# mrjoshuak/go-blosc

Hardware: AMD Instinct MI355X
Metric: GB/s compress+decompress, 1 GiB float32 Shuffle+LZ4 (higher is better)
Workload: dtype u8; 1 GPU; 1024 MiB f32 frame per GPU, shuffle=1 typesize=4 + LZ4, compress then decompress, device-resident; index_trailer=True, chunk_bytes=4096, decode_entry=hb_decompress_frame_dev_hdr (header known to the host)

## Files before the change

go-blosc_amd/csrc/hb_lz4_dec.hip:

```cpp
#include "hb_lz4.h"
#include "hb_dec_common.h"

size_t hb_lz4_dec_workspace(size_t n_out) { return 256 + hb_lz4_region_workspace(n_out); }

__device__ __forceinline__ uint32_t ld32(const uint8_t *p) { return ld4u(p); }

__device__ __forceinline__ void dec_plan_check(const uint8_t *__restrict__ index, uint64_t index_bytes, uint64_t n_src, uint64_t cap,
                                               DecPlan *plan, hb_result *result) {
    plan->mode = DEC_SERIAL; plan->fail = 0; plan->nunits = 0; plan->nbytes = 0; plan->post = 0; plan->stride = 1;
    result->status = HB_OK; result->flags = 0; result->bytes = 0; result->total_bytes = 0; result->reserved = 0;
    if (!index || index_bytes < HB_IDX_HDR_BYTES + 2 * HB_IDX_ENTRY) return;
    uint32_t h[8];
    for (int i = 0; i < 8; i++) h[i] = ld32(index + 4 * i);
    if (h[0] != HB_IDX_MAGIC || h[1] != (HB_IDX_VERSION | (HB_IDX_ENTRY << 16))) return;
    if (h[7] != (h[0] ^ h[1] ^ h[2] ^ h[3] ^ h[4] ^ h[5])) return;
    const uint64_t nunits = h[2];
    if (nunits == 0 || HB_IDX_HDR_BYTES + (nunits + 1) * HB_IDX_ENTRY > index_bytes) return;
    if (h[4] != n_src || h[5] > cap) return;
    if (h[3] != HB_CHUNK || nunits != ((uint64_t)h[5] + HB_CHUNK - 1) / HB_CHUNK) return;
    plan->nunits = (uint32_t)nunits;
    plan->nbytes = h[5];
    const uint32_t m = ((uint32_t)nunits + 7u) / 8u;
    uint32_t P = m / 4u + 1u;
    for (;;) {
        uint32_t x = P, y = m;
        while (y) { const uint32_t t = x % y; x = y; y = t; }
        if (x == 1u) break;
        P++;
    }
    plan->stride = P;
    plan->mode = DEC_INDEXED;
}
__global__ void k_dec_plan(const uint8_t *__restrict__ index, uint64_t index_bytes, uint64_t n_src, uint64_t cap,
                           DecPlan *plan, hb_result *result) {
    dec_plan_check(index, index_bytes, n_src, cap, plan, result);
}

#ifndef DEC_IN_WIN
#define DEC_IN_WIN  1536u
#endif
#define DEC_IN_MARGIN 320u
#define DEC_OUT_MAX HB_CHUNK
#ifndef DEC_LEAN
#define DEC_LEAN 1
#endif
#ifndef DEC_WAVES
#define DEC_WAVES 6
#endif

struct DecCtx {
    const uint8_t *src; uint64_t n_src;
    uint8_t *dst;
    const uint8_t *ent;
    DecPlan *plan;
    uint32_t nbytes, nunits;
    int bun4, ush;
};
#if defined(LAB_DEC_FLUSH) && LAB_DEC_FLUSH == 1
#define LAB_FLUSH_USH() do { } while (0)
#elif defined(LAB_DEC_FLUSH) && LAB_DEC_FLUSH == 2
#define LAB_FLUSH_USH() do { for (uint32_t i = lane * 16u; i < outlen; i += 1024u) st16u(dst + d0 + i, *(const u32x4 *)(s_out + i)); } while (0)
#else
#define LAB_FLUSH_USH() do { \
        uint32_t i_ = lane; \
        for (; i_ + 448u < outlen; i_ += 512u) { \
            _Pragma("unroll") for (uint32_t k_ = 0; k_ < 8u; k_++) udst[(size_t)(i_ + 64u * k_) * (uint32_t)ush] = s_out[i_ + 64u * k_]; \
        } \
        for (; i_ < outlen; i_ += 64) udst[(size_t)i_ * (uint32_t)ush] = s_out[i_]; \
    } while (0)
#endif
__device__ __forceinline__ void dec_unit(const DecCtx &c, const uint32_t u, uint8_t *s_in, uint8_t *s_out, uint2 *s_tq, const int lane) {
    const uint8_t *const src = c.src; const uint64_t n_src = c.n_src; uint8_t *const dst = c.dst; const uint8_t *const ent = c.ent;
    DecPlan *const plan = c.plan; const uint32_t nbytes = c.nbytes, nunits = c.nunits; const int bun4 = c.bun4, ush = c.ush;
    const u32x4 e0 = ld16u(ent + 16 * (size_t)u), e1 = ld16u(ent + 16 * (size_t)(u + 1));
#define RFL(x) ((uint32_t)__builtin_amdgcn_readfirstlane((int)(x)))
    const uint32_t s0 = RFL(e0.x), d0 = RFL(e0.y), s1 = RFL(e1.x), d1 = RFL(e1.y), rem1 = RFL(e1.z), tok1 = RFL(e1.w);
    uint32_t rem = RFL(e0.z), tokpos = RFL(e0.w);
    const bool last = (u + 1 == nunits);
    bool ok = s0 <= s1 && s1 <= n_src && d0 <= d1 && d1 <= nbytes && (d1 - d0) <= DEC_OUT_MAX;
    if (u == 0) ok = ok && s0 == 0 && d0 == 0 && rem == HB_IDX_AT_TOKEN;
    if (last) ok = ok && s1 == n_src && d1 == nbytes;
    if (rem != HB_IDX_AT_TOKEN && tokpos >= n_src) ok = false;
    if (bun4 && ((d0 | d1) & 31u)) ok = false;
    const uint32_t ne = ush ? nbytes / (uint32_t)ush : 1u;
    const uint32_t pj = ush ? d0 / ne : 0u;
    if (ush && (pj >= (uint32_t)ush || d1 > (pj + 1u) * ne)) ok = false;
    uint8_t *const udst = ush ? dst + (size_t)(d0 - pj * ne) * (uint32_t)ush + pj : dst + d0;
    if (!ok) { if (lane == 0) atomicExch(&plan->fail, 1u); return; }
    const uint32_t slen = s1 - s0, outlen = d1 - d0;
    const uint8_t *g = src + s0;

    if (rem != HB_IDX_AT_TOKEN && rem >= outlen) {
        const uint32_t left = rem - outlen;
        bool fine = slen == outlen;
        if (last) fine = fine && left == 0 && (RFL((uint32_t)src[tokpos]) & 15u) == 0u; else fine = fine && rem1 == left && tok1 == tokpos;
        if (!fine) { if (lane == 0) atomicExch(&plan->fail, 1u); return; }
        if (ush) {
            for (uint32_t i = lane * 16u; i < outlen; i += 1024u) {
                if (i + 16u <= outlen) *(u32x4 *)(s_out + i) = ld16u(g + i);
                else for (uint32_t r = i; r < outlen; r++) s_out[r] = g[r];
            }
            wave_sync();
            LAB_FLUSH_USH();
            wave_sync();
        }
        else if (!bun4) wave_copy_g2g(dst + d0, g, outlen, lane);
        else {
            for (uint32_t w = lane; w < outlen / 32u; w += 64) {
                u32x4 oa, ob;
                bitshuffle4_window<true>(ld16u(g + 32u * w), ld16u(g + 32u * w + 16u), oa, ob);
                st16u(dst + d0 + 32u * w, oa);
                st16u(dst + d0 + 32u * w + 16u, ob);
            }
        }
        return;
    }

    const uint32_t sh = (uint32_t)((uintptr_t)g & 15u);
    uint32_t wlo = 0, staged = 0;
    int shw = 0;
    auto stage = [&](const uint32_t at) __attribute__((always_inline)) {
        wave_sync();
        const uint32_t a16 = (sh + at) & ~15u;
        const uint32_t avail = sh + slen - a16;
        const uint32_t cnt = avail < DEC_IN_WIN ? avail : DEC_IN_WIN;
        const u32x4 *ga = (const u32x4 *)(g - sh + a16);
        const uint32_t nv = (cnt + 15u) >> 4;
        for (uint32_t i = lane; i < nv; i += 64) ((u32x4 *)s_in)[i] = ga[i];
        wlo = a16 > sh ? a16 - sh : 0u;
        staged = a16 + cnt - sh;
        shw = (int)sh - (int)a16;
        wave_sync();
    };
    stage(0u);
    uint32_t tok = 0;
    if (rem != HB_IDX_AT_TOKEN) tok = RFL((uint32_t)src[tokpos]);
#define INB(i) s_in[(uint32_t)((int)(i) + shw)]
    uint32_t si = 0, di = 0;
    bool at_token = false;
    bool done = false;

    int slow = 1;
    uint32_t nq = 0;
    uint32_t last_ntok = DEC_BPERM_MIN; (void)last_ntok;
    if (rem == HB_IDX_AT_TOKEN) { rem = 0; slow = 0; }
    while (ok && !done) {
        if (slow) {
            if (slow == 2) {
                if (si >= slen) { ok = false; break; }
                tokpos = s0 + si;
                tok = RFL((uint32_t)((si >= wlo && si < staged) ? INB(si) : g[si]));
                si++;
                rem = tok >> 4;
                if (rem == 15u && !dec_read_ext(s_in, shw, wlo, staged, g, slen, si, rem, lane)) { ok = false; break; }
            }
            slow = 0;
            {
                const uint32_t take = min(rem, outlen - di);
                if (take > slen - si) { ok = false; break; }
                if (si >= wlo && si + take <= staged) { for (uint32_t i = lane; i < take; i += 64) s_out[di + i] = INB(si + i); }
                else { for (uint32_t i = lane; i < take; i += 64) s_out[di + i] = g[si + i]; }
                si += take; di += take; rem -= take;
            }
            if (rem > 0 || di == outlen) { at_token = false; done = true; break; }
            if (slen - si < 2) { ok = false; break; }
            const uint32_t b0 = RFL((uint32_t)((si >= wlo && si < staged) ? INB(si) : g[si]));
            const uint32_t b1 = RFL((uint32_t)((si + 1 >= wlo && si + 1 < staged) ? INB(si + 1) : g[si + 1]));
            const uint32_t offset = b0 | (b1 << 8);
            si += 2;
            uint32_t mlen = (tok & 15u) + 4u;
            if ((tok & 15u) == 15u && !dec_read_ext(s_in, shw, wlo, staged, g, slen, si, mlen, lane)) { ok = false; break; }
            if (offset == 0 || offset > di || mlen > outlen - di) { ok = false; break; }
            dec_match_copy(s_out, di, offset, mlen, lane);
            di += mlen;
            if (si >= wlo && si + 4u <= staged && di < outlen) {
                const uint32_t t2 = RFL((uint32_t)INB(si)), l2 = t2 >> 4;
                if (l2 < 15u && (t2 & 15u) == 15u) {
                    const uint32_t op = si + 1u + l2;
                    if (op + 3u <= staged && RFL((uint32_t)INB(op + 2u)) == 255u) slow = 2;
                }
            }
            continue;
        }
        if (nq == 0u && staged < slen && si + DEC_IN_MARGIN > staged) {
            stage(si);
        }
#if DEC_LEAN
        const bool stop = dec_fill_lean(s_in, (uint32_t)shw, staged, slen, si, nq, s_tq, lane, last_ntok);
        bool rewound = false;
        ok = dec_drain<true>(s_in, shw, s_out, outlen, 0u, di, si, nq, s_tq, stop, rewound, lane);
#else
        const bool stop = dec_fill(s_in, (uint32_t)shw, staged, slen, si, nq, s_tq, lane);
        bool rewound = false;
        ok = dec_drain(s_in, shw, s_out, outlen, 0u, di, si, nq, s_tq, stop, rewound, lane);
#endif
        if (!ok) break;
        if (rewound) { slow = 2; continue; }
        if (stop) {
            if (si == slen || di == outlen) { at_token = true; done = true; }
            else if (staged < slen && si + DEC_IN_MARGIN > staged) continue;
            else slow = 2;
        }
    }
    if (ok) {
        ok = (si == slen) && (di == outlen);
        if (last) ok = ok && (at_token || (rem == 0 && (tok & 15u) == 0u));
        else if (at_token) ok = ok && rem1 == HB_IDX_AT_TOKEN;
        else ok = ok && rem1 == rem && tok1 == tokpos;
    }
    if (!ok) { if (lane == 0) atomicExch(&plan->fail, 1u); wave_sync(); return; }
    wave_sync();
    if (bun4) {
        for (uint32_t w = lane; w < outlen / 32u; w += 64) {
            u32x4 oa, ob;
            bitshuffle4_window<true>(((const u32x4 *)s_out)[2 * w], ((const u32x4 *)s_out)[2 * w + 1], oa, ob);
            ((u32x4 *)s_out)[2 * w] = oa;
            ((u32x4 *)s_out)[2 * w + 1] = ob;
        }
        wave_sync();
    }
    if (ush) {
        LAB_FLUSH_USH();
    } else {
        uint8_t *o = dst + d0;
        uint32_t head = (uint32_t)((16u - ((uintptr_t)o & 15u)) & 15u);
        if (head > outlen) head = outlen;
        if ((uint32_t)lane < head) o[lane] = s_out[lane];
        const uint32_t body = (outlen - head) >> 4;
        if (head == 0) { for (uint32_t i = lane; i < body; i += 64) *(u32x4 *)(o + i * 16u) = *(const u32x4 *)(s_out + i * 16u); }
        else {
            for (uint32_t i = lane; i < body; i += 64) {
                const uint8_t *q = s_out + head + i * 16u;
                u32x4 v;
                v.x = (uint32_t)q[0] | ((uint32_t)q[1] << 8) | ((uint32_t)q[2] << 16) | ((uint32_t)q[3] << 24);
                v.y = (uint32_t)q[4] | ((uint32_t)q[5] << 8) | ((uint32_t)q[6] << 16) | ((uint32_t)q[7] << 24);
                v.z = (uint32_t)q[8] | ((uint32_t)q[9] << 8) | ((uint32_t)q[10] << 16) | ((uint32_t)q[11] << 24);
                v.w = (uint32_t)q[12] | ((uint32_t)q[13] << 8) | ((uint32_t)q[14] << 16) | ((uint32_t)q[15] << 24);
                *(u32x4 *)(o + head + i * 16u) = v;
            }
        }
        const uint32_t done_b = head + body * 16u;
        if (done_b + lane < outlen) o[done_b + lane] = s_out[done_b + lane];
    }
    wave_sync();
}

__global__ __launch_bounds__(64) __attribute__((amdgpu_waves_per_eu(DEC_WAVES))) void k_dec_indexed(const uint8_t *__restrict__ src, uint64_t n_src,
                                                    uint8_t *__restrict__ dst, const uint8_t *__restrict__ index,
                                                    DecPlan *plan, int bun4, int ush, uint32_t plane_mask) {
    __shared__ __attribute__((aligned(16))) uint8_t s_in[DEC_IN_WIN + 128];
    __shared__ __attribute__((aligned(16))) uint8_t s_out[DEC_OUT_MAX + 64];
    __shared__ __attribute__((aligned(16))) uint2 s_tq[DEC_LEAN ? DTQ / 4 : DTQ];
    if (plan->mode != DEC_INDEXED) return;
    const int lane = threadIdx.x;
    const uint32_t nunits = plan->nunits;
    const uint8_t *ent = index + HB_IDX_HDR_BYTES;
    const uint32_t nbytes = plan->nbytes;

    const uint32_t P = plan->stride;
    const uint32_t mgrp = (nunits + 7u) / 8u;
    for (uint32_t it = blockIdx.x; it < mgrp * 8u; it += gridDim.x) {
        uint32_t u = (uint32_t)(((uint64_t)(it >> 3) * P) % mgrp) * 8u + ((it + (it >> 3)) & 7u);
        const bool fused_order = ush && nunits % (uint32_t)ush == 0u && (gridDim.x % (8u * (uint32_t)ush) == 0u || gridDim.x >= nunits);
        if (fused_order ? it >= nunits : u >= nunits) continue;
        if (fused_order) {
            const uint32_t T = (uint32_t)ush, nblk = nunits / T;
            const uint32_t grp = it / (8u * T), r = it % (8u * T);
            uint32_t b = grp * 8u + (r & 7u), j = ((r >> 3) + it / gridDim.x) % T;
            if (grp * 8u + 8u > nblk) {
                const uint32_t k = it - grp * 8u * T, nb = nblk - grp * 8u;
                b = grp * 8u + k % nb; j = k / nb;
            }
            u = j * nblk + b;
            if (!((plane_mask >> j) & 1u)) continue;
        }
        DecCtx c; c.src = src; c.n_src = n_src; c.dst = dst; c.ent = ent; c.plan = plan; c.nbytes = nbytes; c.nunits = nunits; c.bun4 = bun4; c.ush = ush;
        dec_unit(c, u, s_in, s_out, s_tq, lane);
    }
}

__global__ __launch_bounds__(64) void k_bt_dec_plan(const DecBatchFrame *__restrict__ bf, uint32_t nframes, uint32_t *__restrict__ unit_frame, uint32_t total_units) {
    const uint32_t f = blockIdx.x;
    const DecBatchFrame b = bf[f];
    const uint32_t next = f + 1 < nframes ? bf[f + 1].unit0 : total_units;
    __shared__ uint32_t s_mode;
    if (threadIdx.x == 0) {
        dec_plan_check(b.preset == 1 ? b.index : nullptr, b.index_bytes, b.n_src, (uint64_t)b.nbytes, b.plan, b.result);
        b.plan->pad[0] = 0; b.plan->pad[1] = 0;
        if (b.plan->mode == DEC_INDEXED && (b.plan->nunits != b.nunits || b.plan->nbytes != b.nbytes)) b.plan->mode = DEC_SERIAL;
        s_mode = b.plan->mode;
    }
    __syncthreads();
    const bool indexed = s_mode == DEC_INDEXED;
    for (uint32_t u = threadIdx.x; u < next - b.unit0; u += 64) unit_frame[b.unit0 + u] = (u < b.nunits && indexed) ? f : 0xFFFFFFFFu;
}

__global__ __launch_bounds__(64) __attribute__((amdgpu_waves_per_eu(DEC_WAVES))) void k_dec_indexed_batch(const DecBatchFrame *__restrict__ bf,
                                                    const uint32_t *__restrict__ unit_frame, uint32_t total_units) {
    __shared__ __attribute__((aligned(16))) uint8_t s_in[DEC_IN_WIN + 128];
    __shared__ __attribute__((aligned(16))) uint8_t s_out[DEC_OUT_MAX + 64];
    __shared__ __attribute__((aligned(16))) uint2 s_tq[DEC_LEAN ? DTQ / 4 : DTQ];
    const int lane = threadIdx.x;
    for (uint32_t it = blockIdx.x; it < total_units; it += gridDim.x) {
        const uint32_t fid = unit_frame[it];
        if (fid == 0xFFFFFFFFu) continue;
        const DecBatchFrame &f = bf[fid];
        DecCtx c; c.src = f.src; c.n_src = f.n_src; c.dst = f.dst; c.ent = f.index + HB_IDX_HDR_BYTES; c.plan = f.plan;
        c.nbytes = f.nbytes; c.nunits = f.nunits; c.bun4 = f.bun4; c.ush = f.ush;
        uint32_t u = it - f.unit0;
        if (c.ush) {
            const uint32_t T = (uint32_t)c.ush, nblk = c.nunits / T;
            const uint32_t grp = u / (8u * T), r = u % (8u * T);
            uint32_t b = grp * 8u + (r & 7u), j = ((r >> 3) + it / gridDim.x) % T;
            if (grp * 8u + 8u > nblk) { const uint32_t k = u - grp * 8u * T, nb = nblk - grp * 8u; b = grp * 8u + k % nb; j = k / nb; }
            u = j * nblk + b;
        }
        if (u >= c.nunits) continue;
        dec_unit(c, u, s_in, s_out, s_tq, lane);
    }
}

size_t hb_lz4_dec_batch_units(int nframes, const DecBatchFrame *h, uint32_t *unit0_out) {
    uint64_t units = 0;
    for (int k = 0; k < nframes; k++) {
        const uint32_t g = h[k].ush ? 8u * (uint32_t)h[k].ush : 8u;
        units = (units + g - 1) / g * g;
        unit0_out[k] = (uint32_t)units;
        units += h[k].nunits;
    }
    return (size_t)((units + 7) / 8 * 8);
}

int hb_launch_lz4_decode_batch_indexed(int nframes, const DecBatchFrame *d_bf, uint32_t *d_unit_frame, uint32_t total_units, int any_ush, hipStream_t s) {
    hb_prof_begin("k_dec_plan", s);
    hipLaunchKernelGGL(k_bt_dec_plan, dim3((unsigned)nframes), dim3(64), 0, s, d_bf, (uint32_t)nframes, d_unit_frame, total_units);
    hb_prof_end(s);
    if (total_units) {
        unsigned grid = total_units < 256u * 256u ? total_units : 256u * 256u;
        if (any_ush && total_units > 256u * 16u) {
            const unsigned gran = 32u;
            unsigned g2 = total_units / (unsigned)any_ush / gran * gran;
            if (total_units > 256u * 64u && g2 < 256u * 64u) g2 = 256u * 64u;
            if (g2 > 256u * 256u) g2 = 256u * 256u;
            if (g2) grid = g2;
        }
        hb_prof_begin("k_dec_indexed", s);
        hipLaunchKernelGGL(k_dec_indexed_batch, dim3(grid), dim3(64), 0, s, d_bf, (const uint32_t *)d_unit_frame, total_units);
        hb_prof_end(s);
    }
    HB_HIP_TRY(hipGetLastError());
    return HB_OK;
}


__global__ __launch_bounds__(64) void k_dec_serial(const uint8_t *__restrict__ src, uint64_t n_src,
                                                   uint8_t *__restrict__ dst, uint64_t cap, DecPlan *plan,
                                                   hb_result *result, int frame, uint32_t expect, int mark_post) {
    __shared__ __attribute__((aligned(16))) uint8_t s_win[SER_WIN + 128];
    __shared__ __attribute__((aligned(16))) uint8_t s_img[SER_HIST + SER_PAGE + 1024];
    __shared__ __attribute__((aligned(16))) uint2 s_tq[DTQ];
    const int lane = threadIdx.x;
    if (plan->mode == DEC_INDEXED && !plan->fail) {
        if (lane == 0) {
            const uint64_t got = plan->nbytes;
            result->flags = 1; result->bytes = got; result->total_bytes = got;
            result->status = (frame && got != expect) ? HB_ERR_SIZE_MISMATCH : HB_OK;
        }
        return;
    }
    if (mark_post && lane == 0) plan->post = 1;
    int err;
    const uint64_t got = dec_serial_core(src, n_src, dst, cap, s_win, s_img, s_tq, lane, err);
    if (lane == 0) {
        result->flags = 0; result->total_bytes = 0;
        if (err) { result->status = HB_ERR_DECOMPRESSION_FAILED; result->bytes = 0; }
        else if (frame && got != expect) { result->status = HB_ERR_SIZE_MISMATCH; result->bytes = got; }
        else { result->status = HB_OK; result->bytes = got; }
    }
}

__global__ void k_set_result(hb_result *result, int status, uint64_t bytes) {
    result->status = status; result->flags = 0; result->bytes = bytes; result->total_bytes = bytes; result->reserved = 0;
}

int hb_launch_lz4_decode(const hb_dec_args &a, hipStream_t s) {
    if (a.memcpy_payload) {
        if (a.n != a.expect) {
            hipLaunchKernelGGL(k_set_result, dim3(1), dim3(1), 0, s, a.result, HB_ERR_SIZE_MISMATCH, (uint64_t)a.n);
        } else {
            if (a.n) HB_HIP_TRY(hipMemcpyAsync(a.dst, a.src, a.n, hipMemcpyDeviceToDevice, s));
            hipLaunchKernelGGL(k_set_result, dim3(1), dim3(1), 0, s, a.result, HB_OK, (uint64_t)a.n);
        }
        HB_HIP_TRY(hipGetLastError());
        return HB_OK;
    }
    DecPlan *plan = (DecPlan *)a.work;
    const uint8_t *index = a.index;
    size_t index_bytes = a.index_bytes;
    if (hb_lz4_region_wanted(a)) {
        const int rc = hb_launch_lz4_region_index(a, &index, &index_bytes, s);
        if (rc) return rc;
    }
    hb_prof_begin("k_dec_plan", s);
    hipLaunchKernelGGL(k_dec_plan, dim3(1), dim3(1), 0, s, index, (uint64_t)index_bytes, (uint64_t)a.n,
                       (uint64_t)a.cap, plan, a.result);
    hb_prof_end(s);
    if (index) {
        const uint64_t units = (a.cap + HB_CHUNK - 1) / HB_CHUNK;
        const uint64_t units8 = (units + 7) / 8 * 8;
        unsigned grid = (unsigned)(units8 < 8 ? 8 : (units8 < 256u * 256u ? units8 : 256u * 256u));
        if (a.fused_unshuffle_ts && units > 256u * 16u) {
            const unsigned gran = 8u * (unsigned)a.fused_unshuffle_ts;
            unsigned g2 = (unsigned)(units / (uint64_t)a.fused_unshuffle_ts) / gran * gran;
            if (units > 256u * 64u && g2 < 256u * 64u) g2 = 256u * 64u;
            if (g2 > 256u * 256u) g2 = 256u * 256u;
            if (g2) grid = g2;
        }
        hb_prof_begin("k_dec_indexed", s);
        hipLaunchKernelGGL(k_dec_indexed, dim3(grid), dim3(64), 0, s, a.src, (uint64_t)a.n, a.dst, index, plan,
                           a.fused_bitunshuffle4, a.fused_unshuffle_ts, hb_dbg_plane_mask());
        hb_prof_end(s);
    }
    const int fused_any = a.fused_bitunshuffle4 || a.fused_unshuffle_ts;
    uint8_t *serial_dst = fused_any ? a.staged : a.dst;
    if (hb_lz4_region_wanted(a) && a.sym_work) {
        const int rc = hb_launch_lz4_sym_decode(a, serial_dst, a.sym_work, fused_any, s);
        if (rc) return rc;
    }
    hb_prof_begin("k_dec_serial", s);
    hipLaunchKernelGGL(k_dec_serial, dim3(1), dim3(64), 0, s, a.src, (uint64_t)a.n, serial_dst, (uint64_t)a.cap, plan,
                       a.result, a.frame, a.expect, fused_any);
    hb_prof_end(s);
    if (fused_any) {
        const int rc = a.fused_bitunshuffle4
                           ? hb_launch_filter_gated(HB_OP_BITUNSHUFFLE, a.dst, a.staged, a.expect, 4, &plan->post, s)
                           : hb_launch_filter_gated(HB_OP_UNSHUFFLE, a.dst, a.staged, a.expect, a.fused_unshuffle_ts, &plan->post, s);
        if (rc) return rc;
    }
    HB_HIP_TRY(hipGetLastError());
    return HB_OK;
}
```

Before: 389.5 GB/s.

## Add per-block unshuffle decode kernel with coalesced transposed flush for typesize 2/4

Adds a specialized decode kernel where one wave decodes all T byte-planes of a block in turn. The first T-1 planes go to a staging buffer and the last stays in LDS, and the wave then writes the interleaved output with byte-perm transposes and 16-byte stores. This replaces the strided single-byte scatter that each unit used to do for unshuffle. The cost is an extra write and read of T-1 planes through global staging, and less parallelism because each wave now serialises T units.

Measured after the change: 398.2 GB/s (median of 6 runs). 2.2% higher.

```diff
diff --git a/go-blosc_amd/csrc/hb_lz4_dec.hip b/go-blosc_amd/csrc/hb_lz4_dec.hip
--- a/go-blosc_amd/csrc/hb_lz4_dec.hip
+++ b/go-blosc_amd/csrc/hb_lz4_dec.hip
@@ -60,6 +60,14 @@
 #define LAB_FLUSH_USH() do { } while (0)
 #elif defined(LAB_DEC_FLUSH) && LAB_DEC_FLUSH == 2
 #define LAB_FLUSH_USH() do { for (uint32_t i = lane * 16u; i < outlen; i += 1024u) st16u(dst + d0 + i, *(const u32x4 *)(s_out + i)); } while (0)
+#elif defined(LAB_DEC_FLUSH) && LAB_DEC_FLUSH == 3
+#define LAB_FLUSH_USH() do { \
+        uint32_t i_ = lane; \
+        for (; i_ + 448u < outlen; i_ += 512u) { \
+            _Pragma("unroll") for (uint32_t k_ = 0; k_ < 8u; k_++) dst[d0 + i_ + 64u * k_] = s_out[i_ + 64u * k_]; \
+        } \
+        for (; i_ < outlen; i_ += 64) dst[d0 + i_] = s_out[i_]; \
+    } while (0)
 #else
 #define LAB_FLUSH_USH() do { \
         uint32_t i_ = lane; \
@@ -69,7 +77,15 @@
         for (; i_ < outlen; i_ += 64) udst[(size_t)i_ * (uint32_t)ush] = s_out[i_]; \
     } while (0)
 #endif
-__device__ __forceinline__ void dec_unit(const DecCtx &c, const uint32_t u, uint8_t *s_in, uint8_t *s_out, uint2 *s_tq, const int lane) {
+__device__ __forceinline__ void dec_flush_strided(uint8_t *const dst, const uint32_t nbytes, const int ush, const uint32_t d0, const uint32_t outlen,
+                                                  const uint8_t *s_out, const int lane) {
+    const uint32_t ne = nbytes / (uint32_t)ush, pj = d0 / ne;
+    uint8_t *const udst = dst + (size_t)(d0 - pj * ne) * (uint32_t)ush + pj; (void)udst;
+    LAB_FLUSH_USH();
+}
+
+__device__ __forceinline__ bool dec_unit(const DecCtx &c, const uint32_t u, uint8_t *s_in, uint8_t *s_out, uint2 *s_tq, const int lane,
+                                         uint32_t &d0_out, uint32_t &outlen_out) {
     const uint8_t *const src = c.src; const uint64_t n_src = c.n_src; uint8_t *const dst = c.dst; const uint8_t *const ent = c.ent;
     DecPlan *const plan = c.plan; const uint32_t nbytes = c.nbytes, nunits = c.nunits; const int bun4 = c.bun4, ush = c.ush;
     const u32x4 e0 = ld16u(ent + 16 * (size_t)u), e1 = ld16u(ent + 16 * (size_t)(u + 1));
@@ -85,23 +101,21 @@
     const uint32_t ne = ush ? nbytes / (uint32_t)ush : 1u;
     const uint32_t pj = ush ? d0 / ne : 0u;
     if (ush && (pj >= (uint32_t)ush || d1 > (pj + 1u) * ne)) ok = false;
-    uint8_t *const udst = ush ? dst + (size_t)(d0 - pj * ne) * (uint32_t)ush + pj : dst + d0;
-    if (!ok) { if (lane == 0) atomicExch(&plan->fail, 1u); return; }
+    if (!ok) { if (lane == 0) atomicExch(&plan->fail, 1u); return false; }
     const uint32_t slen = s1 - s0, outlen = d1 - d0;
+    d0_out = d0; outlen_out = outlen;
     const uint8_t *g = src + s0;
 
     if (rem != HB_IDX_AT_TOKEN && rem >= outlen) {
         const uint32_t left = rem - outlen;
         bool fine = slen == outlen;
         if (last) fine = fine && left == 0 && (RFL((uint32_t)src[tokpos]) & 15u) == 0u; else fine = fine && rem1 == left && tok1 == tokpos;
-        if (!fine) { if (lane == 0) atomicExch(&plan->fail, 1u); return; }
+        if (!fine) { if (lane == 0) atomicExch(&plan->fail, 1u); return false; }
         if (ush) {
             for (uint32_t i = lane * 16u; i < outlen; i += 1024u) {
                 if (i + 16u <= outlen) *(u32x4 *)(s_out + i) = ld16u(g + i);
                 else for (uint32_t r = i; r < outlen; r++) s_out[r] = g[r];
             }
-            wave_sync();
-            LAB_FLUSH_USH();
             wave_sync();
         }
         else if (!bun4) wave_copy_g2g(dst + d0, g, outlen, lane);
@@ -113,7 +127,7 @@
                 st16u(dst + d0 + 32u * w + 16u, ob);
             }
         }
-        return;
+        return true;
     }
 
     const uint32_t sh = (uint32_t)((uintptr_t)g & 15u);
@@ -208,7 +222,7 @@
         else if (at_token) ok = ok && rem1 == HB_IDX_AT_TOKEN;
         else ok = ok && rem1 == rem && tok1 == tokpos;
     }
-    if (!ok) { if (lane == 0) atomicExch(&plan->fail, 1u); wave_sync(); return; }
+    if (!ok) { if (lane == 0) atomicExch(&plan->fail, 1u); wave_sync(); return false; }
     wave_sync();
     if (bun4) {
         for (uint32_t w = lane; w < outlen / 32u; w += 64) {
@@ -219,9 +233,7 @@
         }
         wave_sync();
     }
-    if (ush) {
-        LAB_FLUSH_USH();
-    } else {
+    if (!ush) {
         uint8_t *o = dst + d0;
         uint32_t head = (uint32_t)((16u - ((uintptr_t)o & 15u)) & 15u);
         if (head > outlen) head = outlen;
@@ -243,6 +255,7 @@
         if (done_b + lane < outlen) o[done_b + lane] = s_out[done_b + lane];
     }
     wave_sync();
+    return true;
 }
 
 __global__ __launch_bounds__(64) __attribute__((amdgpu_waves_per_eu(DEC_WAVES))) void k_dec_indexed(const uint8_t *__restrict__ src, uint64_t n_src,
@@ -275,9 +288,93 @@
             if (!((plane_mask >> j) & 1u)) continue;
         }
         DecCtx c; c.src = src; c.n_src = n_src; c.dst = dst; c.ent = ent; c.plan = plan; c.nbytes = nbytes; c.nunits = nunits; c.bun4 = bun4; c.ush = ush;
-        dec_unit(c, u, s_in, s_out, s_tq, lane);
-    }
-}
+        uint32_t d0, outlen;
+        if (dec_unit(c, u, s_in, s_out, s_tq, lane, d0, outlen) && ush) {
+            dec_flush_strided(dst, nbytes, ush, d0, outlen, s_out, lane);
+            wave_sync();
+        }
+    }
+}
+
+
+__device__ __forceinline__ u32x4 ush_transpose4(const uint32_t p0, const uint32_t p1, const uint32_t p2, const uint32_t p3) {
+    const uint32_t lo01 = __builtin_amdgcn_perm(p1, p0, 0x05010400u), hi01 = __builtin_amdgcn_perm(p1, p0, 0x07030602u);
+    const uint32_t lo23 = __builtin_amdgcn_perm(p3, p2, 0x05010400u), hi23 = __builtin_amdgcn_perm(p3, p2, 0x07030602u);
+    u32x4 o;
+    o.x = __builtin_amdgcn_perm(lo23, lo01, 0x05040100u); o.y = __builtin_amdgcn_perm(lo23, lo01, 0x07060302u);
+    o.z = __builtin_amdgcn_perm(hi23, hi01, 0x05040100u); o.w = __builtin_amdgcn_perm(hi23, hi01, 0x07060302u);
+    return o;
+}
+
+template <int T>
+__device__ __forceinline__ void dec_flush_block(uint8_t *__restrict__ dst, const uint8_t *__restrict__ staged, const uint8_t *img, const uint32_t nblk,
+                                                const uint32_t b, const int lane) {
+    const uint8_t *pl = staged + (size_t)b * HB_CHUNK;
+    const size_t ps = (size_t)nblk * HB_CHUNK;
+    uint8_t *o = dst + (size_t)b * (HB_CHUNK * T);
+#pragma unroll
+    for (uint32_t r = 0; r < HB_CHUNK / 1024u; r++) {
+        const uint32_t e = r * 1024u + (uint32_t)lane * 16u;
+        u32x4 p[T];
+#pragma unroll
+        for (int j = 0; j < T - 1; j++) p[j] = *(const u32x4 *)(pl + j * ps + e);
+        p[T - 1] = *(const u32x4 *)(img + e);
+        if constexpr (T == 4) {
+            st16u(o + 4u * e, ush_transpose4(p[0].x, p[1].x, p[2].x, p[3].x));
+            st16u(o + 4u * e + 16u, ush_transpose4(p[0].y, p[1].y, p[2].y, p[3].y));
+            st16u(o + 4u * e + 32u, ush_transpose4(p[0].z, p[1].z, p[2].z, p[3].z));
+            st16u(o + 4u * e + 48u, ush_transpose4(p[0].w, p[1].w, p[2].w, p[3].w));
+        } else {
+            u32x4 a, c;
+            a.x = __builtin_amdgcn_perm(p[1].x, p[0].x, 0x05010400u); a.y = __builtin_amdgcn_perm(p[1].x, p[0].x, 0x07030602u);
+            a.z = __builtin_amdgcn_perm(p[1].y, p[0].y, 0x05010400u); a.w = __builtin_amdgcn_perm(p[1].y, p[0].y, 0x07030602u);
+            c.x = __builtin_amdgcn_perm(p[1].z, p[0].z, 0x05010400u); c.y = __builtin_amdgcn_perm(p[1].z, p[0].z, 0x07030602u);
+            c.z = __builtin_amdgcn_perm(p[1].w, p[0].w, 0x05010400u); c.w = __builtin_amdgcn_perm(p[1].w, p[0].w, 0x07030602u);
+            st16u(o + 2u * e, a);
+            st16u(o + 2u * e + 16u, c);
+        }
+    }
+}
+
+template <int T>
+__global__ __launch_bounds__(64) __attribute__((amdgpu_waves_per_eu(DEC_WAVES))) void k_dec_indexed_ush(const uint8_t *__restrict__ src, uint64_t n_src,
+                                                    uint8_t *__restrict__ dst, uint8_t *__restrict__ staged, const uint8_t *__restrict__ index,
+                                                    DecPlan *plan, uint32_t plane_mask) {
+    __shared__ __attribute__((aligned(16))) uint8_t s_in[DEC_IN_WIN + 128];
+    __shared__ __attribute__((aligned(16))) uint8_t s_out[DEC_OUT_MAX + 64];
+    __shared__ __attribute__((aligned(16))) uint2 s_tq[DEC_LEAN ? DTQ / 4 : DTQ];
+    if (plan->mode != DEC_INDEXED) return;
+    const int lane = threadIdx.x;
+    const uint32_t nunits = plan->nunits, nbytes = plan->nbytes;
+    DecCtx c; c.src = src; c.n_src = n_src; c.dst = dst; c.ent = index + HB_IDX_HDR_BYTES; c.plan = plan; c.nbytes = nbytes; c.nunits = nunits;
+    c.bun4 = 0; c.ush = T;
+    const bool blocked = nunits % (uint32_t)T == 0u && nbytes == nunits * HB_CHUNK;
+    const uint32_t nblk = (nunits + (uint32_t)T - 1u) / (uint32_t)T;
+    const bool flush = blocked && (plane_mask & ((1u << T) - 1u)) == (1u << T) - 1u;
+    for (uint32_t b = blockIdx.x; b < nblk; b += gridDim.x) {
+        bool ok = true;
+#pragma nounroll
+        for (uint32_t j = 0; j < (uint32_t)T; j++) {
+            const uint32_t u = blocked ? j * nblk + b : b * (uint32_t)T + j;
+            if (u >= nunits || (blocked && !((plane_mask >> j) & 1u))) continue;
+            uint32_t d0, outlen;
+            const bool oku = dec_unit(c, u, s_in, s_out, s_tq, lane, d0, outlen);
+            ok = ok && oku;
+            if (oku && flush && j + 1u < (uint32_t)T) {
+                uint8_t *st = staged + (size_t)u * HB_CHUNK;
+#pragma unroll
+                for (uint32_t r = 0; r < HB_CHUNK / 1024u; r++)
+                    *(u32x4 *)(st + r * 1024u + (uint32_t)lane * 16u) = *(const u32x4 *)(s_out + r * 1024u + (uint32_t)lane * 16u);
+            } else if (oku && !blocked) {
+                dec_flush_strided(dst, nbytes, T, d0, outlen, s_out, lane);
+            }
+            if (j + 1u < (uint32_t)T) wave_sync();
+        }
+        if (flush && ok) dec_flush_block<T>(dst, staged, s_out, nblk, b, lane);
+        wave_sync();
+    }
+}
+
 
 __global__ __launch_bounds__(64) void k_bt_dec_plan(const DecBatchFrame *__restrict__ bf, uint32_t nframes, uint32_t *__restrict__ unit_frame, uint32_t total_units) {
     const uint32_t f = blockIdx.x;
@@ -316,7 +413,11 @@
             u = j * nblk + b;
         }
         if (u >= c.nunits) continue;
-        dec_unit(c, u, s_in, s_out, s_tq, lane);
+        uint32_t d0, outlen;
+        if (dec_unit(c, u, s_in, s_out, s_tq, lane, d0, outlen) && c.ush) {
+            dec_flush_strided(c.dst, c.nbytes, c.ush, d0, outlen, s_out, lane);
+            wave_sync();
+        }
     }
 }
 
@@ -417,8 +518,14 @@
             if (g2) grid = g2;
         }
         hb_prof_begin("k_dec_indexed", s);
-        hipLaunchKernelGGL(k_dec_indexed, dim3(grid), dim3(64), 0, s, a.src, (uint64_t)a.n, a.dst, index, plan,
-                           a.fused_bitunshuffle4, a.fused_unshuffle_ts, hb_dbg_plane_mask());
+        const int T = a.fused_unshuffle_ts;
+        if ((T == 2 || T == 4) && units > 256u * 16u) {
+            if (T == 2) hipLaunchKernelGGL(k_dec_indexed_ush<2>, dim3(grid), dim3(64), 0, s, a.src, (uint64_t)a.n, a.dst, a.staged, index, plan, hb_dbg_plane_mask());
+            else hipLaunchKernelGGL(k_dec_indexed_ush<4>, dim3(grid), dim3(64), 0, s, a.src, (uint64_t)a.n, a.dst, a.staged, index, plan, hb_dbg_plane_mask());
+        } else {
+            hipLaunchKernelGGL(k_dec_indexed, dim3(grid), dim3(64), 0, s, a.src, (uint64_t)a.n, a.dst, index, plan,
+                               a.fused_bitunshuffle4, a.fused_unshuffle_ts, hb_dbg_plane_mask());
+        }
         hb_prof_end(s);
     }
     const int fused_any = a.fused_bitunshuffle4 || a.fused_unshuffle_ts;
```
